# koide3/gtsam_points

Measured on AMD Instinct MI355X. Metric: point-correspondences/sec (VGICP linearize, 1M-pt source vs 2M-pt voxel map), higher is better.
Workload: dtype f64; 1 GPU; BASELINE configs[1]: single VGICP factor per GPU, 1M synthetic source pts vs 2M-pt GaussianVoxel; target_points=2000000, num_voxels=73733, num_buckets=262144, device_warmup_steps=14074

## Files before the change

gtsam_points_amd/csrc/gp_vgicp.hip:

```cpp
#include <algorithm>
#include <atomic>
#include <chrono>
#include <cmath>
#include <cstdlib>
#include <cstring>

#include "gp_host.hpp"
#include "gp_vgicp_tile.hpp"
#include "gp_vgicp_tile2.hpp"
#include "gp_vgicp_finalize.hpp"
#include "gp_vgicp_stream.hpp"

namespace gp {



template <int MODE>
struct ModeTraits {
  static constexpr int kAcc = MODE == MODE_ERR ? 2 : (MODE == MODE_LIN ? ACC_SIZE : ACCG_SIZE);
  static constexpr int kStride = MODE == MODE_LIN_GENERAL ? ACCG_STRIDE : ACC_STRIDE;
};

template <int MODE>
__device__ __forceinline__ void accumulate_point(const FactorDesc& f, const Pose& Tl, const Pose& Te, int i, double* acc) {
// ... 699 lines not shown
  return per * gp::kNumXCD;
}

bool poses_are_rigid(const double* poses_host, size_t F) {
  if (!poses_host) return false;
  for (size_t i = 0; i < F; i++)
    if (!gp::pose_is_rigid(poses_host + 16 * i)) return false;
  return true;
}

template <int MODE>
int launch_tiles(gp_vgicp_batch* b, const PoseSource& ps, double* partials) {
  if (b->num_tiles <= 0) return GP_OK;
  const int fam = MODE == gp::MODE_LIN_GENERAL ? GP_KERNEL_REFERENCE : b->family;
  const bool single_plan = b->planned;
  const int chunk = (fam == GP_KERNEL_REFERENCE || single_plan || (fam == GP_KERNEL_STREAM && ps.inl.use)) ? 0 : b->tuning.xcd_chunk;
  const dim3 grid_dim(grid_tiles(b->num_tiles, chunk)), block(gp::kBlockThreads);
  const gp::FactorDesc* fd = b->d_factors.as<gp::FactorDesc>();
  const gp::TileDesc* td = b->d_tiles.as<gp::TileDesc>();
  gp::InlinePoses inl = ps.inl;
  inl.stagger = b->tuning.stagger;
  inl.xcd_chunk = chunk;
  inl.tile_points = b->tile_points;
  inl.plan = b->plan;
  inl.trace = b->trace;
  const bool traced = b->trace != nullptr && inl.use && MODE == gp::MODE_LIN;
#define GP_ARGS grid_dim, block, 0, b->stream, fd, td, b->num_tiles, ps.d_lin, ps.d_eval, inl, partials
  if constexpr (MODE == gp::MODE_LIN_GENERAL) {
    hipLaunchKernelGGL(gp::vgicp_tile_kernel<MODE>, GP_ARGS);
  } else if (fam == GP_KERNEL_REFERENCE) {
    hipLaunchKernelGGL(gp::vgicp_tile_kernel<MODE>, GP_ARGS);
  } else if (fam == GP_KERNEL_STREAM) {
#define GP_LAUNCH_STREAM(NT, INL, SV, PK, TRACE) hipLaunchKernelGGL((gp::vgicp_stream_kernel<MODE, NT, INL, SV, PK, TRACE>), GP_ARGS)
#define GP_LAUNCH_STREAM_S(INL, SV)                                  \
  do {                                                               \
    if (b->packed) {                                                 \
      if (b->nt) GP_LAUNCH_STREAM(true, INL, SV, true, false);       \
      else GP_LAUNCH_STREAM(false, INL, SV, true, false);            \
    } else {                                                         \
      if (b->nt) GP_LAUNCH_STREAM(true, INL, SV, false, false);      \
      else GP_LAUNCH_STREAM(false, INL, SV, false, false);           \
    }                                                                \
  } while (0)
    if (traced && !b->any_sv) {
      if constexpr (MODE == gp::MODE_LIN) {
        if (b->packed) {
          if (b->nt) GP_LAUNCH_STREAM(true, true, false, true, true);
          else GP_LAUNCH_STREAM(false, true, false, true, true);
        } else {
          if (b->nt) GP_LAUNCH_STREAM(true, true, false, false, true);
          else GP_LAUNCH_STREAM(false, true, false, false, true);
        }
      }
    } else if (inl.use && MODE == gp::MODE_LIN && b->tuning.experiment && b->planned && b->packed && b->nt && !b->any_sv) {
      if constexpr (MODE == gp::MODE_LIN) {
        if (b->tuning.experiment == 1) hipLaunchKernelGGL((gp::vgicp_stream_kernel<MODE, true, true, false, true, false, 1>), GP_ARGS);
        else hipLaunchKernelGGL((gp::vgicp_stream_kernel<MODE, true, true, false, true, false, 2>), GP_ARGS);
      }
    } else if (inl.use) {
      if (b->any_sv) GP_LAUNCH_STREAM_S(true, true);
      else GP_LAUNCH_STREAM_S(true, false);
    } else {
      if (b->any_sv) GP_LAUNCH_STREAM_S(false, true);
      else GP_LAUNCH_STREAM_S(false, false);
    }
#undef GP_LAUNCH_STREAM_S
#undef GP_LAUNCH_STREAM
  } else {
#define GP_LAUNCH_PIPE(F32, PPT, GRID, LEAN, AHEAD) hipLaunchKernelGGL((gp::vgicp_pipeline_kernel<MODE, F32, PPT, GRID, false, LEAN, AHEAD>), GP_ARGS)
    if (fam == GP_KERNEL_HASHED) {
      GP_LAUNCH_PIPE(true, 4, false, false, false);
    } else if (fam == GP_KERNEL_GRID_F64) {
      GP_LAUNCH_PIPE(false, 4, true, false, false);
    } else {
      if constexpr (MODE == gp::MODE_LIN) GP_LAUNCH_PIPE(true, 4, true, true, true);
      else GP_LAUNCH_PIPE(true, 4, true, true, false);
    }
#undef GP_LAUNCH_PIPE
  }
#undef GP_ARGS
  GP_HIP(hipGetLastError());
  return GP_OK;
}

template <bool GENERAL>
int launch_finalize(gp_vgicp_batch* b, const PoseSource& ps, const double* partials, gp_linearized6* out_dev, gp::DoneFlags done = {}, int parts = 1) {
  if constexpr (GENERAL) {
    hipLaunchKernelGGL(gp::vgicp_finalize_kernel<true>, dim3((int)b->factors.size()), dim3(gp::kFinalizeThreads), 0, b->stream, b->d_factors.as<gp::FactorDesc>(),
                       ps.d_lin, ps.inl, partials, out_dev, done);
  } else {
    constexpr bool narrow = true;
    const int nparts = parts < 0 ? -parts : parts;
    if (nparts > 1 && narrow)
      hipLaunchKernelGGL(gp::vgicp_finalize_rigid_kernel<256>, dim3((int)b->factors.size() * nparts), dim3(256), 0, b->stream, b->d_factors.as<gp::FactorDesc>(), ps.d_lin,
                         ps.inl, partials, out_dev, done, parts);
    else
      hipLaunchKernelGGL(gp::vgicp_finalize_rigid_kernel<gp::kFinalizeThreads>, dim3((int)b->factors.size() * nparts), dim3(gp::kFinalizeThreads), 0, b->stream,
                         b->d_factors.as<gp::FactorDesc>(), ps.d_lin, ps.inl, partials, out_dev, done, parts);
  }
  GP_HIP(hipGetLastError());
  return GP_OK;
}

int launch_linearize(gp_vgicp_batch* b, const PoseSource& ps, gp_linearized6* out_dev, bool rigid, gp::DoneFlags done = {}, int parts = 1, bool timed = false) {
  if (b->factors.empty()) return GP_OK;
  double* partials = nullptr;
  GP_TRY(partials_ptr(b, &partials));
// ... 63 lines not shown
    b->tuning = f->tuning;
    const int rc = build_table(b);
    if (rc != GP_OK) {
      delete b;
      return rc;
    }
    f->self_batch = b;
  }
  if (table_is_stale(f->self_batch)) GP_TRY(build_table(f->self_batch));
  return GP_OK;
}

}

extern "C" {

static int apply_tuning(gp_vgicp_tuning* t, int key, int value) {
  switch (key) {
    case GP_TUNE_KERNEL:
      if (value != GP_KERNEL_REFERENCE && value != GP_KERNEL_HASHED && value != GP_KERNEL_GRID_F64 && value != GP_KERNEL_LOOKAHEAD && value != GP_KERNEL_STREAM)
        return gp::fail(GP_ERROR_INVALID_ARGUMENT, "GP_TUNE_KERNEL: one of GP_KERNEL_REFERENCE (0), _HASHED (2), _GRID_F64 (3), _LOOKAHEAD (8), _STREAM (12)");
      t->kernel = value;
      return GP_OK;
    case GP_TUNE_SOURCE_POLICY:
      if (value < 0 || value > 2) return gp::fail(GP_ERROR_INVALID_ARGUMENT, "GP_TUNE_SOURCE_POLICY: 0 (per batch), 1 (default cache policy), 2 (non-temporal)");
      t->source_policy = value;
      return GP_OK;
    case GP_TUNE_XCD_CHUNK:
      if (value < 0 || value > 4096) return gp::fail(GP_ERROR_INVALID_ARGUMENT, "GP_TUNE_XCD_CHUNK: 0 (contiguous eighths) .. 4096 tiles per run");
      t->xcd_chunk = value;
      return GP_OK;
    case GP_TUNE_STAGGER:
      if (value < 0 || value > 64) return gp::fail(GP_ERROR_INVALID_ARGUMENT, "GP_TUNE_STAGGER: 0..64 (x 512 clocks)");
      t->stagger = value;
      return GP_OK;
    case GP_TUNE_TILE_INTERLEAVE:
      t->tile_interleave = value ? 1 : 0;
      return GP_OK;
    case GP_TUNE_FUSED_FINALIZE:
      t->fused_finalize = value ? 1 : 0;
      return GP_OK;
    case GP_TUNE_MAX_WORKGROUPS:
      if (value < 8 || value > 1024) return gp::fail(GP_ERROR_INVALID_ARGUMENT, "GP_TUNE_MAX_WORKGROUPS: 8 .. 1024");
      t->max_wgs = value;
      return GP_OK;
    case GP_TUNE_TILE_CHUNKS:
      if (value < 0 || value > 64) return gp::fail(GP_ERROR_INVALID_ARGUMENT, "GP_TUNE_TILE_CHUNKS: 0 (automatic) .. 64 chunks per wave");
      t->tile_chunks = value;
      return GP_OK;
    case GP_TUNE_SOURCE_MIRROR:
      t->source_mirror = value ? 1 : 0;
      return GP_OK;
    case GP_TUNE_EXPERIMENT:
      if (value < 0 || value > 2) return gp::fail(GP_ERROR_INVALID_ARGUMENT, "GP_TUNE_EXPERIMENT: 0 (off), 1 (block-grid warm-up), 2 (f32 covariance rotation: breaks parity, timing only)");
      t->experiment = value;
      return GP_OK;
    case GP_TUNE_BALANCE:
      if (value < -1 || value > 600) return gp::fail(GP_ERROR_INVALID_ARGUMENT, "GP_TUNE_BALANCE: -1 (automatic), 0 (flat) .. 600 (per mille of the mean share per dispatch round)");
      t->balance = value;
      return GP_OK;
    default:
      if (key >= GP_TUNE_XCD_WEIGHT_0 && key < GP_TUNE_XCD_WEIGHT_0 + 8) {
        if (value < 500 || value > 1500) return gp::fail(GP_ERROR_INVALID_ARGUMENT, "GP_TUNE_XCD_WEIGHT_x: 500..1500 (per mille of the mean share)");
        t->xcd_weights[key - GP_TUNE_XCD_WEIGHT_0] = value;
        t->xcd_weights_set = true;
        return GP_OK;
      }
      return gp::fail(GP_ERROR_INVALID_ARGUMENT, "unknown GP_TUNE_* key");
  }
}

int gp_vgicp_batch_set_tuning(gp_vgicp_batch_t* b, int key, int value) {
  if (!b) return gp::fail(GP_ERROR_INVALID_ARGUMENT, "gp_vgicp_batch_set_tuning: null batch");
  if (key == GP_TUNE_TIMING) {
    b->timing = value != 0;
    return GP_OK;
  }
  if (key == GP_TUNE_TEST_ARRIVAL_SKEW) {
    b->arrived[0] += (unsigned long long)(value > 0 ? value : 0);
    if (b->d_factor_arrive.ptr && value > 0) {
      const unsigned long long v = 1ull << 40;
      GP_HIP(hipStreamSynchronize(b->stream));
      GP_HIP(hipMemcpy(b->d_factor_arrive.ptr, &v, sizeof(v), hipMemcpyHostToDevice));
    }
    return GP_OK;
  }
  GP_TRY(apply_tuning(&b->tuning, key, value));
  b->table_dirty = true;
  return GP_OK;
}

int gp_vgicp_batch_get_tuning(const gp_vgicp_batch_t* b, int key, int* value) {
  if (!b || !value) return gp::fail(GP_ERROR_INVALID_ARGUMENT, "gp_vgicp_batch_get_tuning: null");
  switch (key) {
    case GP_TUNE_KERNEL: *value = b->tuning.kernel; return GP_OK;
    case GP_TUNE_SOURCE_POLICY: *value = b->tuning.source_policy; return GP_OK;
    case GP_TUNE_XCD_CHUNK: *value = b->tuning.xcd_chunk; return GP_OK;
    case GP_TUNE_STAGGER: *value = b->tuning.stagger; return GP_OK;
    case GP_TUNE_TILE_INTERLEAVE: *value = b->tuning.tile_interleave; return GP_OK;
    case GP_TUNE_BALANCE: *value = b->tuning.balance; return GP_OK;
    case GP_TUNE_FUSED_FINALIZE: *value = b->tuning.fused_finalize; return GP_OK;
    case GP_TUNE_TILE_CHUNKS: *value = b->tuning.tile_chunks; return GP_OK;
    case GP_TUNE_EFFECTIVE_KERNEL: *value = b->table_dirty ? -1 : b->family; return GP_OK;
    case GP_TUNE_SOURCE_MIRROR: *value = b->tuning.source_mirror; return GP_OK;
    case GP_TUNE_EXPERIMENT: *value = b->tuning.experiment; return GP_OK;
    case GP_TUNE_EFFECTIVE_MIRROR: *value = b->table_dirty ? -1 : (b->packed ? 1 : 0); return GP_OK;
    default: return gp::fail(GP_ERROR_INVALID_ARGUMENT, "unknown GP_TUNE_* key");
// ... 756 lines not shown
```

gtsam_points_amd/csrc/gp_vgicp_stream.hpp:

```cpp
#pragma once

#include "gp_vgicp_finalize.hpp"
#include "gp_vgicp_tile2.hpp"

namespace gp {

template <bool NT>
__device__ __forceinline__ void chunk_dma12_row(const GP_GLOBAL char* urow, unsigned voff, char* slot) {
  chunk_dma12_pts<NT>(urow, voff, slot);
}

template <int N>
__device__ __forceinline__ void vm_wait_blk_n(v4i& blk) {
  static_assert(N == 0 || N == 3 || N == 4 || N == 5, "counts of the stream schedule");
  if constexpr (N == 0) asm volatile("s_waitcnt vmcnt(0)" : "+v"(blk) : : "memory");
  if constexpr (N == 3) asm volatile("s_waitcnt vmcnt(3)" : "+v"(blk) : : "memory");
  if constexpr (N == 4) asm volatile("s_waitcnt vmcnt(4)" : "+v"(blk) : : "memory");
  if constexpr (N == 5) asm volatile("s_waitcnt vmcnt(5)" : "+v"(blk) : : "memory");
}

struct WaveWork {
  size_t first;
  int n;
  int tail;
// ... 36 lines not shown
  for (int t0 = slice; t0 < row_count && wave < 4; t0 += 32 * kSlices) {
    double v[32];
#pragma unroll
    for (int k = 0; k < 32; k++) {
      const int t = t0 + k * kSlices;
      v[k] = t < row_count ? __builtin_bit_cast(double, __hip_atomic_load(base + (size_t)t * ACC_STRIDE, __ATOMIC_RELAXED, __HIP_MEMORY_SCOPE_AGENT)) : 0.0;
    }
#pragma unroll
    for (int w = 16; w > 0; w >>= 1) {
#pragma unroll
      for (int k = 0; k < w; k++) v[k] += v[k + w];
    }
    total += v[0];
  }
  total += __shfl_xor(total, 32, 64);
  if (tr && threadIdx.x == 0) tr[14] = __builtin_amdgcn_s_memrealtime();
  if (lane < 32 && wave < 4) wsum[wave * 32 + lane] = total;
  __syncthreads();
  if (wave != 0) return;
  double s = lane < 32 ? (wsum[lane] + wsum[64 + lane]) + (wsum[32 + lane] + wsum[96 + lane]) : 0.0;
  if (lane == 32) s = __builtin_bit_cast(double, t_rows);
  if (lane == 33) s = __builtin_bit_cast(double, __builtin_amdgcn_s_memrealtime());
  if (lane < 34) asm volatile("global_store_dwordx2 %0, %1, off sc0 sc1" : : "v"(out + lane), "v"(s) : "memory");
  asm volatile("s_waitcnt vmcnt(0)" ::: "memory");
  if (lane == 0) asm volatile("global_store_dwordx2 %0, %1, off sc0 sc1" : : "v"(flag), "v"(seq) : "memory");
  if (tr && lane == 0) tr[15] = __builtin_amdgcn_s_memrealtime();
}

__device__ __forceinline__ void finalize_part_error(const double* __restrict__ partials, const int row_begin, const int row_count, double* wsum, double* out,
                                                    unsigned long long* flag, const unsigned long long seq) {
  const int lane = threadIdx.x & 63, wave = threadIdx.x >> 6;
  const unsigned long long* base = reinterpret_cast<const unsigned long long*>(partials + (size_t)row_begin * ACC_STRIDE + ACC_ERR);
  double s = 0.0;
  for (int t = threadIdx.x; t < row_count && wave < 4; t += 256)
    s += __builtin_bit_cast(double, __hip_atomic_load(base + (size_t)t * ACC_STRIDE, __ATOMIC_RELAXED, __HIP_MEMORY_SCOPE_AGENT));
#pragma unroll
  for (int off = 32; off > 0; off >>= 1) s += __shfl_down(s, off, 64);
  if (lane == 0 && wave < 4) wsum[wave] = s;
  __syncthreads();
  if (threadIdx.x != 0) return;
  const double total = (wsum[0] + wsum[1]) + (wsum[2] + wsum[3]);
  asm volatile("global_store_dwordx2 %0, %1, off sc0 sc1\n\ts_waitcnt vmcnt(0)" : : "v"(out), "v"(total) : "memory");
  asm volatile("global_store_dwordx2 %0, %1, off sc0 sc1" : : "v"(flag), "v"(seq) : "memory");
}

template <int MODE, bool NT, bool INL, bool SV, bool PK, bool TRACE = false, int EXP = 0, int W = 4>
__global__ void __launch_bounds__(64 * W, 4) vgicp_stream_kernel(const FactorDesc* __restrict__ factors, const TileDesc* __restrict__ tiles, int num_tiles,
                                                               const double* __restrict__ poses_lin, const double* __restrict__ poses_eval, const InlinePoses inl,
                                                               double* __restrict__ partials) {
  static_assert(MODE == MODE_LIN || MODE == MODE_ERR, "rigid linearise and error evaluation");
  constexpr int NACC = MODE == MODE_ERR ? 2 : 32;
  constexpr int KC = PK ? 2 : 3;
  constexpr int K = 1 + KC + (SV ? 1 : 0);
  constexpr int kNrmSlotBytes = SV ? kPtsSlotBytes : 0;
  constexpr int kChunkSlotBytes = PK ? kCovSlotBytes : kPtsSlotBytes + kCovSlotBytes;
  constexpr int kRingBytes = 2 * kChunkSlotBytes + 2 * kNrmSlotBytes;
  constexpr int kWaveBytes = kRingBytes > kWaveLdsBytes ? kRingBytes : kWaveLdsBytes;
  static_assert(kWaveBytes >= kWaveLdsBytes, "the reduction needs 8.5 KB of the wave's region");
  static_assert(W * kWaveBytes <= 160 * 1024, "one workgroup's rings must fit the compute unit's LDS");
  __shared__ __attribute__((aligned(16))) char smem[W * kWaveBytes];
  const unsigned long long t_begin = INL ? __builtin_amdgcn_s_memrealtime() : 0ull;
  const int bx = blockIdx.x % kNumXCD, bq = blockIdx.x / kNumXCD;
  int tile_idx;
  FactorDesc f;
  WaveWork ww;
  int factor_idx = 0, row;
  int wgs_per_xcd = 0;
  const int wave = __builtin_amdgcn_readfirstlane(threadIdx.x >> 6);
  if constexpr (INL) {
    PlanFields pf = plan_fields(inl.plan, bx, bq);
    wgs_per_xcd = pf.gx;
    int tile_points = inl.tile_points, fn = inl.factor.n;
    const float* fpts = inl.factor.points;
    const float* fcov = inl.factor.covs;
    const float* fnrm = inl.factor.normals;
    const char* fpk = inl.factor.packed;
    asm volatile("" : "+s"(pf.nr), "+s"(pf.pre), "+s"(pf.lo), "+s"(pf.extra), "+s"(pf.xbegin), "+s"(pf.L), "+s"(pf.before_last), "+s"(pf.gx), "+s"(pf.tail), "+s"(tile_points),
                 "+s"(fn), "+s"(fpts), "+s"(fcov), "+s"(fnrm), "+s"(fpk));
    int begin, count;
    if (tile_points == 0) {
      tile_idx = bx * pf.gx + bq;
      plan_tile(pf, bx, bq, &begin, &count);
    } else {
      const int per = (num_tiles + kNumXCD - 1) / kNumXCD;
      tile_idx = bx * per + bq;
      if (bq >= per || tile_idx >= num_tiles) return;
      begin = tile_idx * tile_points;
      count = min(tile_points, fn - begin);
    }
    f = inl.factor;
    f.points = fpts;
    f.covs = fcov;
    f.normals = fnrm;
    f.packed = fpk;
    row = tile_idx;
    ww = split_tile<W>(begin, count, wave);
  } else {
    if (inl.xcd_chunk > 0) {
      const int c = inl.xcd_chunk;
      tile_idx = ((bq / c) * kNumXCD + bx) * c + (bq % c);
    } else {
      const int per = (num_tiles + kNumXCD - 1) / kNumXCD;
      tile_idx = bx * per + bq;
    }
    if (tile_idx >= num_tiles) return;
    const TileDesc tile = tiles[tile_idx];
    f = factors[tile.factor];
    factor_idx = tile.factor;
    row = tile.row;
    ww = split_tile<W>(__builtin_amdgcn_readfirstlane(tile.begin), __builtin_amdgcn_readfirstlane(tile.count), wave);
  }
  unsigned long long* trace = TRACE ? inl.trace : nullptr;
  GP_TRACE(0);
  if constexpr (INL && MODE == MODE_LIN) {
    if (inl.arrive && inl.rows_per_part > 0 && blockIdx.x < kNumXCD && threadIdx.x == 0)
      asm volatile("global_store_dwordx2 %0, %1, off sc0 sc1" : : "v"(inl.fin_out + (size_t)blockIdx.x * inl.fin_stride + 34), "v"(t_begin) : "memory");
  }
  if constexpr (TRACE) {
    if (trace && threadIdx.x == 0) {
      trace[(size_t)tile_idx * 16 + 10] = __builtin_amdgcn_s_memrealtime();
      trace[(size_t)tile_idx * 16 + 8] = __builtin_amdgcn_s_getreg(GP_GETREG_HW_ID);
      trace[(size_t)tile_idx * 16 + 9] = __builtin_amdgcn_s_getreg(GP_GETREG_XCC_ID);
    }
  }
  const int lane = threadIdx.x & 63;
  const int n = __builtin_amdgcn_readfirstlane(ww.n);
  const int tail = __builtin_amdgcn_readfirstlane(ww.tail);
  const size_t first = ww.first;
  char* wbase = smem + wave * kWaveBytes;
  auto pslot = [&](int par) { return PK ? wbase + par * kCovSlotBytes : wbase + par * kPtsSlotBytes; };
  auto nslot = [&](int par) { return PK ? wbase + 2 * kCovSlotBytes + par * kNrmSlotBytes : wbase + 2 * kPtsSlotBytes + par * kNrmSlotBytes; };
  auto cslot = [&](int par) { return PK ? wbase + par * kCovSlotBytes : wbase + 2 * kPtsSlotBytes + 2 * kNrmSlotBytes + par * kCovSlotBytes; };
  const GP_GLOBAL char* upts = PK ? uniform_ptr((const GP_GLOBAL char*)f.packed + (first >> 6) * (size_t)kPackedChunkBytes) : uniform_ptr((const GP_GLOBAL char*)as_global(f.points) + 12 * first);
  const GP_GLOBAL char* ucov = PK ? upts : uniform_ptr((const GP_GLOBAL char*)as_global(f.covs) + 36 * first);
  const GP_GLOBAL char* unrm = SV ? uniform_ptr((const GP_GLOBAL char*)as_global(f.normals) + 12 * first) : nullptr;
  const unsigned voff = (unsigned)lane * 12u;
  constexpr size_t kSrcChunkStride = PK ? (size_t)kPackedChunkBytes : (size_t)kChunkPoints * 12, kCovChunkStride = PK ? (size_t)kPackedChunkBytes : (size_t)kChunkPoints * 36;
  auto dma_head = [&](int j, int par) {
    chunk_dma12_pts<NT>(upts + (size_t)j * kSrcChunkStride, voff, pslot(par));
    if constexpr (SV) chunk_dma12_row<NT>(unrm + (size_t)j * (kChunkPoints * 12), voff, nslot(par));
  };
  auto dma_cov = [&](int j, int par) {
    if constexpr (PK) chunk_dma12_cov_packed<NT>(ucov + (size_t)j * kCovChunkStride, voff, cslot(par));
    else chunk_dma12_cov<NT>(ucov + (size_t)j * kCovChunkStride, voff, cslot(par));
  };

  if (n > 0) dma_head(0, 0);

  const Pose Tl = INL ? load_pose(inl.lin) : load_pose(poses_lin + 16 * (size_t)factor_idx);
  const Pose Te = MODE == MODE_ERR ? (INL ? load_pose(inl.eval) : load_pose(poses_eval + 16 * (size_t)factor_idx)) : Tl;
  const double leaf = uniform_f64(f.map.leaf), inv_leaf = uniform_f64(f.map.inv_leaf), half_leaf = uniform_f64(0.5 * f.map.leaf);
  const int glo0 = f.map.glo[0], glo1 = f.map.glo[1], glo2 = f.map.glo[2];
  const unsigned gd0 = __builtin_amdgcn_readfirstlane((unsigned)f.map.gdim[0]), gd1 = __builtin_amdgcn_readfirstlane((unsigned)f.map.gdim[1]), gd2 = (unsigned)f.map.gdim[2];
  const GP_GLOBAL char* gblocks = uniform_ptr((const GP_GLOBAL char*)f.map.gblocks);
  const GP_GLOBAL char* records = uniform_ptr((const GP_GLOBAL char*)f.map.records);

  v4i warm = {0, 0, 0, 0};
  if constexpr (EXP == 1) {
    const unsigned gbytes = gd0 * gd1 * gd2 * 16u;
#pragma unroll
    for (int k = 0; k < 4; k++) {
      const unsigned off = ((unsigned)(k * wgs_per_xcd + bq) * 256u + threadIdx.x) * 16u;
      if (off < gbytes) asm volatile("global_load_dwordx4 %0, %1, %2" : "+v"(warm) : "v"(off), "s"(gblocks) : "memory");
    }
  }
  double tvx, tvy, tvz;
  asm volatile("v_mov_b64 %0, %1" : "=v"(tvx) : "s"(Tl.tx));
  asm volatile("v_mov_b64 %0, %1" : "=v"(tvy) : "s"(Tl.ty));
  asm volatile("v_mov_b64 %0, %1" : "=v"(tvz) : "s"(Tl.tz));

  float acc[NACC];
#pragma unroll
  for (int k = 0; k < NACC; k++) acc[k] = 0.f;

  struct Ahead {
    v4i blk;
    float ex, ey, ez, qx, qy, qz;
    int pos;
  };
  auto front = [&](float pxf, float pyf, float pzf, float nxf, float nyf, float nzf, bool active, Ahead& P) {
#pragma clang fp contract(off)
    const double dx = (double)pxf, dy = (double)pyf, dz = (double)pzf;
    const double lx = __builtin_fma(Tl.r00, dx, __builtin_fma(Tl.r01, dy, __builtin_fma(Tl.r02, dz, tvx)));
    const double ly = __builtin_fma(Tl.r10, dx, __builtin_fma(Tl.r11, dy, __builtin_fma(Tl.r12, dz, tvy)));
    const double lz = __builtin_fma(Tl.r20, dx, __builtin_fma(Tl.r21, dy, __builtin_fma(Tl.r22, dz, tvz)));
    const double ux = lx * inv_leaf, uy = ly * inv_leaf, uz = lz * inv_leaf;
    const int cx = (int)__builtin_floor(ux), cy = (int)__builtin_floor(uy), cz = (int)__builtin_floor(uz);
    if constexpr (MODE == MODE_ERR) {
      const double ex_ = __builtin_fma(Te.r00, dx, __builtin_fma(Te.r01, dy, __builtin_fma(Te.r02, dz, Te.tx)));
      const double ey_ = __builtin_fma(Te.r10, dx, __builtin_fma(Te.r11, dy, __builtin_fma(Te.r12, dz, Te.ty)));
      const double ez_ = __builtin_fma(Te.r20, dx, __builtin_fma(Te.r21, dy, __builtin_fma(Te.r22, dz, Te.tz)));
      P.ex = (float)(__builtin_fma(-leaf, __builtin_amdgcn_fract(ux), half_leaf) + (lx - ex_));
      P.ey = (float)(__builtin_fma(-leaf, __builtin_amdgcn_fract(uy), half_leaf) + (ly - ey_));
      P.ez = (float)(__builtin_fma(-leaf, __builtin_amdgcn_fract(uz), half_leaf) + (lz - ez_));
      P.qx = P.qy = P.qz = 0.f;
    } else {
      P.ex = (float)__builtin_fma(-leaf, __builtin_amdgcn_fract(ux), half_leaf);
      P.ey = (float)__builtin_fma(-leaf, __builtin_amdgcn_fract(uy), half_leaf);
      P.ez = (float)__builtin_fma(-leaf, __builtin_amdgcn_fract(uz), half_leaf);
      P.qx = (float)lx;
      P.qy = (float)ly;
      P.qz = (float)lz;
    }
    bool live = active && finite3(pxf, pyf, pzf);
    if constexpr (SV) {
      const double nx = (double)nxf, ny = (double)nyf, nz = (double)nzf;
      const double tnx = __builtin_fma(Tl.r02, nz, __builtin_fma(Tl.r01, ny, Tl.r00 * nx)), tny = __builtin_fma(Tl.r12, nz, __builtin_fma(Tl.r11, ny, Tl.r10 * nx));
      const double tnz = __builtin_fma(Tl.r22, nz, __builtin_fma(Tl.r21, ny, Tl.r20 * nx));
      const double s = __builtin_fma(lz, tnz, __builtin_fma(ly, tny, lx * tnx));
      const double qq = __builtin_fma(lz, lz, __builtin_fma(ly, ly, lx * lx));
      if (s > 0.0 && s * s > (0.174 * 0.174) * qq) live = false;
    }
    const unsigned bx = (unsigned)((cx >> 2) - glo0), by = (unsigned)((cy >> 2) - glo1), bz = (unsigned)((cz >> 2) - glo2);
    const bool inbox = (bx < gd0) & (by < gd1) & (bz < gd2);
    const unsigned lin = inbox ? mad24s(mad24s(bz, gd1, by), gd0, bx) : 0u;
    P.pos = (inbox && live) ? (((cz & 3) << 4) | ((cy & 3) << 2) | (cx & 3)) : -1;
    grid_issue_s(gblocks, lin * 16u, P.blk);
  };
  auto front_ring = [&](int par, Ahead& P) {
    const v3f pt = *reinterpret_cast<const v3f*>(pslot(par) + 16 * lane);
    v3f nr = {0.f, 0.f, 0.f};
    if constexpr (SV) nr = *reinterpret_cast<const v3f*>(nslot(par) + 16 * lane);
    front(pt.x, pt.y, pt.z, nr.x, nr.y, nr.z, true, P);
  };
  auto back_issue = [&](const Ahead& P, v4f& head, v2d& c01, v2d& c23, v2d& c45) -> bool {
    const unsigned long long bits = ((unsigned long long)(unsigned)P.blk.y << 32) | (unsigned long long)(unsigned)P.blk.x;
    const int pos = P.pos < 0 ? 0 : P.pos;
    const bool hit = P.pos >= 0 && ((bits >> pos) & 1ull);
    const int idx = P.blk.z + __popcll(bits & ((1ull << pos) - 1ull));
    record_issue_s(records, hit ? (unsigned)idx << 6 : 0u, head, c01, c23, c45);
    return hit;
  };
  auto cov_ring = [&](int par, double* a) {
    if constexpr (PK) {
      const char* c = cslot(par) + 16 * lane;
      const v3f ca = *reinterpret_cast<const v3f*>(c + kPtsSlotBytes), cb = *reinterpret_cast<const v3f*>(c + 2 * kPtsSlotBytes);
      a[0] = (double)ca.x, a[1] = (double)ca.y, a[2] = (double)ca.z, a[3] = (double)cb.x, a[4] = (double)cb.y, a[5] = (double)cb.z;
    } else {
      const char* c = cslot(par) + 48 * lane;
      const v3f c0 = *reinterpret_cast<const v3f*>(c), c1 = *reinterpret_cast<const v3f*>(c + 16), c2 = *reinterpret_cast<const v3f*>(c + 32);
      const float c9[9] = {c0.x, c0.y, c0.z, c1.x, c1.y, c1.z, c2.x, c2.y, c2.z};
      load_cov6(c9, a);
    }
  };

  Ahead Pc;
  v4f head;
  v2d c01, c23, c45;
  double a[6];
  if (n > 0) {
    vm_wait<0>();
    if constexpr (EXP == 1) asm volatile("" : : "v"(warm));
    GP_TRACE(1);
    front_ring(0, Pc);
    dma_cov(0, 0);
    const bool has1 = n > 1;
    if (has1) dma_head(1, 1);
    else vm_wait<KC>();
    vm_wait_blk_n<K>(Pc.blk);
    GP_TRACE(2);
    bool hit = back_issue(Pc, head, c01, c23, c45);
    if (has1) dma_cov(1, 1);
    else asm volatile("s_waitcnt vmcnt(0)" ::: "memory");
    vm_wait_rec<KC>(head, c01, c23, c45);
    for (int j = 0;; j++) {
      const int par = j & 1;
      const bool more = j + 1 < n, more2 = j + 2 < n;
      Ahead Pn;
      if (more) front_ring(par ^ 1, Pn);
      cov_ring(par, a);
      if (more2) {
        asm volatile("s_waitcnt lgkmcnt(0)" ::: "memory");
        dma_head(j + 2, par);
        dma_cov(j + 2, par);
      }
      if (hit) accumulate_core2<MODE, EXP == 2>(Tl, a, c01, c23, c45, Pc.ex + head.x, Pc.ey + head.y, Pc.ez + head.z, Pc.qx, Pc.qy, Pc.qz, acc);
      if constexpr (TRACE) {
        if (j == 0) GP_TRACE(3);
        if (j == 1) GP_TRACE(5);
      }
      if (!more) break;
      if (!more2) asm volatile("s_waitcnt vmcnt(0)" ::: "memory");
      vm_wait_blk_n<K>(Pn.blk);
      if constexpr (TRACE) {
        if (j == 0) GP_TRACE(4);
      }
      hit = back_issue(Pn, head, c01, c23, c45);
      vm_wait_rec<0>(head, c01, c23, c45);
      Pc.ex = Pn.ex;
      Pc.ey = Pn.ey;
      Pc.ez = Pn.ez;
      Pc.qx = Pn.qx;
      Pc.qy = Pn.qy;
      Pc.qz = Pn.qz;
    }
    vm_wait<0>();
  }
  if (tail > 0) {
    const GP_GLOBAL float* points = as_global(f.points);
    const GP_GLOBAL float* covs = as_global(f.covs);
    const bool active = lane < tail;
    const size_t i = first + (size_t)n * kChunkPoints + (active ? lane : 0);
    v3f pt, nr = {0.f, 0.f, 0.f};
    v4f ca, cb;
    float cc;
    asm volatile(
      "global_load_dwordx3 %0, %4, off\n\t"
      "global_load_dwordx4 %1, %5, off\n\t"
      "global_load_dwordx4 %2, %5, off offset:16\n\t"
      "global_load_dword %3, %5, off offset:32\n\t"
      "s_waitcnt vmcnt(0)"
      : "=&v"(pt), "=&v"(ca), "=&v"(cb), "=&v"(cc)
      : "v"(points + 3 * i), "v"(covs + 9 * i)
      : "memory");
    if constexpr (SV) {
      const GP_GLOBAL float* normals = as_global(f.normals);
      asm volatile(
        "global_load_dwordx3 %0, %1, off\n\t"
        "s_waitcnt vmcnt(0)"
        : "=&v"(nr)
        : "v"(normals + 3 * i)
        : "memory");
    }
    const float c9[9] = {ca.x, ca.y, ca.z, ca.w, cb.x, cb.y, cb.z, cb.w, cc};
    Ahead P;
    front(pt.x, pt.y, pt.z, nr.x, nr.y, nr.z, active, P);
    vm_wait_blk_n<0>(P.blk);
    const bool hit = back_issue(P, head, c01, c23, c45);
    vm_wait_rec<0>(head, c01, c23, c45);
    load_cov6(c9, a);
    if (hit) accumulate_core2<MODE>(Tl, a, c01, c23, c45, P.ex + head.x, P.ey + head.y, P.ez + head.z, P.qx, P.qy, P.qz, acc);
  }

  GP_TRACE(6);
  constexpr int kRowStrideF = 66;
  static_assert(32 * kRowStrideF * 4 + 32 * 8 <= kWaveBytes, "f32 transposition buffer + wave sums must fit the wave's LDS region");
  float* wtf = reinterpret_cast<float*>(wbase);
  double* wsums = reinterpret_cast<double*>(wbase + kWaveBytes - 32 * 8);
  if constexpr (MODE == MODE_ERR) {
#pragma unroll
    for (int k = 0; k < 2; k++) {
      double v = (double)acc[k];
#pragma unroll
      for (int off = 32; off > 0; off >>= 1) v += __shfl_xor(v, off, 64);
      if (lane == 0) wsums[k] = v;
    }
  } else {
// ... 130 lines not shown
```

gtsam_points_amd/csrc/gp_vgicp_tile2.hpp:

```cpp
#pragma once

#include "gp_vgicp_tile.hpp"

namespace gp {

template <typename T>
__device__ __forceinline__ const GP_GLOBAL T* uniform_ptr(const GP_GLOBAL T* p) {
  const unsigned long long v = (unsigned long long)p;
  const unsigned lo = __builtin_amdgcn_readfirstlane((unsigned)v), hi = __builtin_amdgcn_readfirstlane((unsigned)(v >> 32));
  return (const GP_GLOBAL T*)(((unsigned long long)hi << 32) | lo);
}
__device__ __forceinline__ double uniform_f64(double x) {
  const unsigned long long v = __builtin_bit_cast(unsigned long long, x);
  const unsigned lo = __builtin_amdgcn_readfirstlane((unsigned)v), hi = __builtin_amdgcn_readfirstlane((unsigned)(v >> 32));
  return __builtin_bit_cast(double, ((unsigned long long)hi << 32) | lo);
}

constexpr int kPtsSlotBytes = 1024, kCovSlotBytes = 3072, kWaveLdsBytes = 8704;
static_assert(2 * kPtsSlotBytes + 2 * kCovSlotBytes <= kWaveLdsBytes, "ring must fit the wave's LDS region");

template <bool NT>
__device__ __forceinline__ void chunk_dma12_pts(const GP_GLOBAL char* upts, unsigned voff, char* pslot) {
  const unsigned lds_pts = (unsigned)(size_t)(GP_LDS char*)pslot;
  unsigned saved;
// ... 55 lines not shown
__device__ __forceinline__ void chunk_dma12_cov_packed(const GP_GLOBAL char* uchunk, unsigned voff, char* slot) {
  const unsigned lds_c1 = (unsigned)(size_t)(GP_LDS char*)slot + 256u, lds_c2 = lds_c1 + 256u;
  unsigned saved;
  if constexpr (NT) {
    asm volatile(
      "s_mov_b32 %0, m0\n\t"
      "s_mov_b32 m0, %3\n\t"
      "global_load_lds_dwordx3 %1, %2 offset:768 nt\n\t"
      "s_mov_b32 m0, %4\n\t"
      "global_load_lds_dwordx3 %1, %2 offset:1536 nt\n\t"
      "s_mov_b32 m0, %0"
      : "=&s"(saved)
      : "v"(voff), "s"(uchunk), "s"(lds_c1), "s"(lds_c2)
      : "memory");
  } else {
    asm volatile(
      "s_mov_b32 %0, m0\n\t"
      "s_mov_b32 m0, %3\n\t"
      "global_load_lds_dwordx3 %1, %2 offset:768\n\t"
      "s_mov_b32 m0, %4\n\t"
      "global_load_lds_dwordx3 %1, %2 offset:1536\n\t"
      "s_mov_b32 m0, %0"
      : "=&s"(saved)
      : "v"(voff), "s"(uchunk), "s"(lds_c1), "s"(lds_c2)
      : "memory");
  }
}

__device__ __forceinline__ unsigned mad24(unsigned a, unsigned b, unsigned c) {
  unsigned r;
  asm("v_mad_u32_u24 %0, %1, %2, %3" : "=v"(r) : "v"(a), "v"(b), "v"(c));
  return r;
}

__device__ __forceinline__ unsigned mad24s(unsigned a, unsigned b_uniform, unsigned c) {
  unsigned r;
  asm("v_mad_u32_u24 %0, %1, %2, %3" : "=v"(r) : "v"(a), "s"(b_uniform), "v"(c));
  return r;
}

__device__ __forceinline__ void grid_issue_s(const GP_GLOBAL char* base, unsigned off, v4i& blk) {
  asm volatile("global_load_dwordx4 %0, %1, %2" : "=&v"(blk) : "v"(off), "s"(base) : "memory");
}
__device__ __forceinline__ void record_issue_s(const GP_GLOBAL char* base, unsigned off, v4f& head, v2d& c01, v2d& c23, v2d& c45) {
  asm volatile(
    "global_load_dwordx4 %0, %4, %5\n\t"
    "global_load_dwordx4 %1, %4, %5 offset:16\n\t"
    "global_load_dwordx4 %2, %4, %5 offset:32\n\t"
    "global_load_dwordx4 %3, %4, %5 offset:48"
    : "=&v"(head), "=&v"(c01), "=&v"(c23), "=&v"(c45)
    : "v"(off), "s"(base)
    : "memory");
}
template <int N>
__device__ __forceinline__ void vm_wait() {
  static_assert(N >= 0 && N <= 8, "counts used by the schedules below");
  if constexpr (N == 0) asm volatile("s_waitcnt vmcnt(0)" ::: "memory");
  if constexpr (N == 1) asm volatile("s_waitcnt vmcnt(1)" ::: "memory");
  if constexpr (N == 2) asm volatile("s_waitcnt vmcnt(2)" ::: "memory");
  if constexpr (N == 3) asm volatile("s_waitcnt vmcnt(3)" ::: "memory");
  if constexpr (N == 4) asm volatile("s_waitcnt vmcnt(4)" ::: "memory");
  if constexpr (N == 7) asm volatile("s_waitcnt vmcnt(7)" ::: "memory");
  static_assert(N == 0 || N == 1 || N == 2 || N == 3 || N == 4 || N == 7, "add the count");
}
template <int N>
__device__ __forceinline__ void vm_wait_blk(v4i& blk) {
  if constexpr (N == 0) asm volatile("s_waitcnt vmcnt(0)" : "+v"(blk) : : "memory");
  if constexpr (N == 1) asm volatile("s_waitcnt vmcnt(1)" : "+v"(blk) : : "memory");
  if constexpr (N == 3) asm volatile("s_waitcnt vmcnt(3)" : "+v"(blk) : : "memory");
  if constexpr (N == 4) asm volatile("s_waitcnt vmcnt(4)" : "+v"(blk) : : "memory");
  static_assert(N == 0 || N == 1 || N == 3 || N == 4, "add the count");
}
template <int N>
__device__ __forceinline__ void vm_wait_rec(v4f& head, v2d& c01, v2d& c23, v2d& c45) {
  if constexpr (N == 0) asm volatile("s_waitcnt vmcnt(0)" : "+v"(head), "+v"(c01), "+v"(c23), "+v"(c45) : : "memory");
  if constexpr (N == 2) asm volatile("s_waitcnt vmcnt(2)" : "+v"(head), "+v"(c01), "+v"(c23), "+v"(c45) : : "memory");
  if constexpr (N == 3) asm volatile("s_waitcnt vmcnt(3)" : "+v"(head), "+v"(c01), "+v"(c23), "+v"(c45) : : "memory");
  if constexpr (N == 4) asm volatile("s_waitcnt vmcnt(4)" : "+v"(head), "+v"(c01), "+v"(c23), "+v"(c45) : : "memory");
  static_assert(N == 0 || N == 2 || N == 3 || N == 4, "add the count");
}

template <int MODE, bool ROT32 = false>
__device__ __forceinline__ void accumulate_core2(const Pose& Tl, const double* a, const v2d& c01, const v2d& c23, const v2d& c45, float RX, float RY, float RZ, float QX,
                                                 float QY, float QZ, float* acc) {
#pragma clang fp contract(off)
  float M0, M1, M2, M3, M4, M5;
  if constexpr (ROT32) {
    const float r00 = (float)Tl.r00, r01 = (float)Tl.r01, r02 = (float)Tl.r02, r10 = (float)Tl.r10, r11 = (float)Tl.r11, r12 = (float)Tl.r12, r20 = (float)Tl.r20,
                r21 = (float)Tl.r21, r22 = (float)Tl.r22;
    const float a00 = (float)a[0], a01 = (float)a[1], a02 = (float)a[2], a11 = (float)a[3], a12 = (float)a[4], a22 = (float)a[5];
    const auto d3 = [](float x0, float y0, float x1, float y1, float x2, float y2) { return __builtin_fmaf(x2, y2, __builtin_fmaf(x1, y1, x0 * y0)); };
    const float rc00 = d3(r00, a00, r01, a01, r02, a02), rc01 = d3(r00, a01, r01, a11, r02, a12), rc02 = d3(r00, a02, r01, a12, r02, a22);
    const float rc10 = d3(r10, a00, r11, a01, r12, a02), rc11 = d3(r10, a01, r11, a11, r12, a12), rc12 = d3(r10, a02, r11, a12, r12, a22);
    const float rc20 = d3(r20, a00, r21, a01, r22, a02), rc21 = d3(r20, a01, r21, a11, r22, a12), rc22 = d3(r20, a02, r21, a12, r22, a22);
    const double s00 = c01.x + (double)d3(rc00, r00, rc01, r01, rc02, r02), s01 = c01.y + (double)d3(rc00, r10, rc01, r11, rc02, r12);
    const double s02 = c23.x + (double)d3(rc00, r20, rc01, r21, rc02, r22), s11 = c23.y + (double)d3(rc10, r10, rc11, r11, rc12, r12);
    const double s12 = c45.x + (double)d3(rc10, r20, rc11, r21, rc12, r22), s22 = c45.y + (double)d3(rc20, r20, rc21, r21, rc22, r22);
    const double i00 = __builtin_fma(s11, s22, -(s12 * s12)), i01 = __builtin_fma(s02, s12, -(s01 * s22)), i02 = __builtin_fma(s01, s12, -(s02 * s11));
    const double det = __builtin_fma(s02, i02, __builtin_fma(s01, i01, s00 * i00));
    double x = __builtin_amdgcn_rcp(det);
    x = x * __builtin_fma(-det, x, 2.0);
    M0 = (float)(i00 * x);
    M1 = (float)(i01 * x);
    M2 = (float)(i02 * x);
    M3 = (float)(__builtin_fma(s00, s22, -(s02 * s02)) * x);
    M4 = (float)(__builtin_fma(s01, s02, -(s00 * s12)) * x);
    M5 = (float)(__builtin_fma(s00, s11, -(s01 * s01)) * x);
  } else {
    const double a00 = a[0], a01 = a[1], a02 = a[2], a11 = a[3], a12 = a[4], a22 = a[5];
    const auto dot3 = [](double x0, double y0, double x1, double y1, double x2, double y2) { return __builtin_fma(x2, y2, __builtin_fma(x1, y1, x0 * y0)); };
    const auto dot3p = [](double c, double x0, double y0, double x1, double y1, double x2, double y2) { return __builtin_fma(x2, y2, __builtin_fma(x1, y1, __builtin_fma(x0, y0, c))); };
    const double rc00 = dot3(Tl.r00, a00, Tl.r01, a01, Tl.r02, a02), rc01 = dot3(Tl.r00, a01, Tl.r01, a11, Tl.r02, a12), rc02 = dot3(Tl.r00, a02, Tl.r01, a12, Tl.r02, a22);
    const double rc10 = dot3(Tl.r10, a00, Tl.r11, a01, Tl.r12, a02), rc11 = dot3(Tl.r10, a01, Tl.r11, a11, Tl.r12, a12), rc12 = dot3(Tl.r10, a02, Tl.r11, a12, Tl.r12, a22);
    const double rc20 = dot3(Tl.r20, a00, Tl.r21, a01, Tl.r22, a02), rc21 = dot3(Tl.r20, a01, Tl.r21, a11, Tl.r22, a12), rc22 = dot3(Tl.r20, a02, Tl.r21, a12, Tl.r22, a22);
    const double s00 = dot3p(c01.x, rc00, Tl.r00, rc01, Tl.r01, rc02, Tl.r02);
    const double s01 = dot3p(c01.y, rc00, Tl.r10, rc01, Tl.r11, rc02, Tl.r12);
// ... 54 lines not shown
```

Measured before the change: 50.22 billion point-correspondences/s.

## Stage voxel record gathers through LDS DMA to overlap with next chunk's loads

```diff
diff --git a/gtsam_points_amd/csrc/gp_vgicp.hip b/gtsam_points_amd/csrc/gp_vgicp.hip
--- a/gtsam_points_amd/csrc/gp_vgicp.hip
+++ b/gtsam_points_amd/csrc/gp_vgicp.hip
@@ -775,7 +775,17 @@
           else GP_LAUNCH_STREAM(false, true, false, false, true);
         }
       }
-    } else if (inl.use && MODE == gp::MODE_LIN && b->tuning.experiment && b->planned && b->packed && b->nt && !b->any_sv) {
+    } else if (b->tuning.experiment == 3 && b->packed && !b->any_sv) {
+#define GP_LAUNCH_UNSTAGED(NT, INL) hipLaunchKernelGGL((gp::vgicp_stream_kernel<MODE, NT, INL, false, true, false, 3>), GP_ARGS)
+      if (inl.use) {
+        if (b->nt) GP_LAUNCH_UNSTAGED(true, true);
+        else GP_LAUNCH_UNSTAGED(false, true);
+      } else {
+        if (b->nt) GP_LAUNCH_UNSTAGED(true, false);
+        else GP_LAUNCH_UNSTAGED(false, false);
+      }
+#undef GP_LAUNCH_UNSTAGED
+    } else if (inl.use && MODE == gp::MODE_LIN && (b->tuning.experiment == 1 || b->tuning.experiment == 2) && b->planned && b->packed && b->nt && !b->any_sv) {
       if constexpr (MODE == gp::MODE_LIN) {
         if (b->tuning.experiment == 1) hipLaunchKernelGGL((gp::vgicp_stream_kernel<MODE, true, true, false, true, false, 1>), GP_ARGS);
         else hipLaunchKernelGGL((gp::vgicp_stream_kernel<MODE, true, true, false, true, false, 2>), GP_ARGS);
@@ -945,7 +955,9 @@
       t->source_mirror = value ? 1 : 0;
       return GP_OK;
     case GP_TUNE_EXPERIMENT:
-      if (value < 0 || value > 2) return gp::fail(GP_ERROR_INVALID_ARGUMENT, "GP_TUNE_EXPERIMENT: 0 (off), 1 (block-grid warm-up), 2 (f32 covariance rotation: breaks parity, timing only)");
+      if (value < 0 || value > 3)
+        return gp::fail(GP_ERROR_INVALID_ARGUMENT, "GP_TUNE_EXPERIMENT: 0 (off), 1 (block-grid warm-up), 2 (f32 covariance rotation: breaks parity, timing only), "
+                                                   "3 (packed stream without the record stage)");
       t->experiment = value;
       return GP_OK;
     case GP_TUNE_BALANCE:
diff --git a/gtsam_points_amd/csrc/gp_vgicp_stream.hpp b/gtsam_points_amd/csrc/gp_vgicp_stream.hpp
--- a/gtsam_points_amd/csrc/gp_vgicp_stream.hpp
+++ b/gtsam_points_amd/csrc/gp_vgicp_stream.hpp
@@ -112,9 +112,10 @@
   constexpr int NACC = MODE == MODE_ERR ? 2 : 32;
   constexpr int KC = PK ? 2 : 3;
   constexpr int K = 1 + KC + (SV ? 1 : 0);
+  constexpr bool STAGE = PK && !SV && EXP != 3;
   constexpr int kNrmSlotBytes = SV ? kPtsSlotBytes : 0;
   constexpr int kChunkSlotBytes = PK ? kCovSlotBytes : kPtsSlotBytes + kCovSlotBytes;
-  constexpr int kRingBytes = 2 * kChunkSlotBytes + 2 * kNrmSlotBytes;
+  constexpr int kRingBytes = 2 * kChunkSlotBytes + 2 * kNrmSlotBytes + (STAGE ? kStageBytes : 0);
   constexpr int kWaveBytes = kRingBytes > kWaveLdsBytes ? kRingBytes : kWaveLdsBytes;
   static_assert(kWaveBytes >= kWaveLdsBytes, "the reduction needs 8.5 KB of the wave's region");
   static_assert(W * kWaveBytes <= 160 * 1024, "one workgroup's rings must fit the compute unit's LDS");
@@ -191,6 +192,7 @@
   auto pslot = [&](int par) { return PK ? wbase + par * kCovSlotBytes : wbase + par * kPtsSlotBytes; };
   auto nslot = [&](int par) { return PK ? wbase + 2 * kCovSlotBytes + par * kNrmSlotBytes : wbase + 2 * kPtsSlotBytes + par * kNrmSlotBytes; };
   auto cslot = [&](int par) { return PK ? wbase + par * kCovSlotBytes : wbase + 2 * kPtsSlotBytes + 2 * kNrmSlotBytes + par * kCovSlotBytes; };
+  char* const stage = wbase + 2 * kChunkSlotBytes;
   const GP_GLOBAL char* upts = PK ? uniform_ptr((const GP_GLOBAL char*)f.packed + (first >> 6) * (size_t)kPackedChunkBytes) : uniform_ptr((const GP_GLOBAL char*)as_global(f.points) + 12 * first);
   const GP_GLOBAL char* ucov = PK ? upts : uniform_ptr((const GP_GLOBAL char*)as_global(f.covs) + 36 * first);
   const GP_GLOBAL char* unrm = SV ? uniform_ptr((const GP_GLOBAL char*)as_global(f.normals) + 12 * first) : nullptr;
@@ -291,6 +293,14 @@
     record_issue_s(records, hit ? (unsigned)idx << 6 : 0u, head, c01, c23, c45);
     return hit;
   };
+  auto back_issue_stage = [&](const Ahead& P) -> bool {
+    const unsigned long long bits = ((unsigned long long)(unsigned)P.blk.y << 32) | (unsigned long long)(unsigned)P.blk.x;
+    const int pos = P.pos < 0 ? 0 : P.pos;
+    const bool hit = P.pos >= 0 && ((bits >> pos) & 1ull);
+    const int idx = P.blk.z + __popcll(bits & ((1ull << pos) - 1ull));
+    record_dma_s(records, hit ? (unsigned)idx << 6 : 0u, stage);
+    return hit;
+  };
   auto cov_ring = [&](int par, double* a) {
     if constexpr (PK) {
       const char* c = cslot(par) + 16 * lane;
@@ -319,40 +329,85 @@
     else vm_wait<KC>();
     vm_wait_blk_n<K>(Pc.blk);
     GP_TRACE(2);
-    bool hit = back_issue(Pc, head, c01, c23, c45);
-    if (has1) dma_cov(1, 1);
-    else asm volatile("s_waitcnt vmcnt(0)" ::: "memory");
-    vm_wait_rec<KC>(head, c01, c23, c45);
-    for (int j = 0;; j++) {
-      const int par = j & 1;
-      const bool more = j + 1 < n, more2 = j + 2 < n;
-      Ahead Pn;
-      if (more) front_ring(par ^ 1, Pn);
-      cov_ring(par, a);
-      if (more2) {
-        asm volatile("s_waitcnt lgkmcnt(0)" ::: "memory");
-        dma_head(j + 2, par);
-        dma_cov(j + 2, par);
-      }
-      if (hit) accumulate_core2<MODE, EXP == 2>(Tl, a, c01, c23, c45, Pc.ex + head.x, Pc.ey + head.y, Pc.ez + head.z, Pc.qx, Pc.qy, Pc.qz, acc);
-      if constexpr (TRACE) {
-        if (j == 0) GP_TRACE(3);
-        if (j == 1) GP_TRACE(5);
-      }
-      if (!more) break;
-      if (!more2) asm volatile("s_waitcnt vmcnt(0)" ::: "memory");
-      vm_wait_blk_n<K>(Pn.blk);
-      if constexpr (TRACE) {
-        if (j == 0) GP_TRACE(4);
-      }
-      hit = back_issue(Pn, head, c01, c23, c45);
-      vm_wait_rec<0>(head, c01, c23, c45);
-      Pc.ex = Pn.ex;
-      Pc.ey = Pn.ey;
-      Pc.ez = Pn.ez;
-      Pc.qx = Pn.qx;
-      Pc.qy = Pn.qy;
-      Pc.qz = Pn.qz;
+    if constexpr (STAGE) {
+      static_assert(K - KC == 1, "the stage schedule counts one head row per chunk (packed stream, no normals)");
+      bool hit = back_issue_stage(Pc);
+      if (has1) dma_cov(1, 1);
+      for (int j = 0;; j++) {
+        const int par = j & 1;
+        const bool more = j + 1 < n, more2 = j + 2 < n;
+        Ahead Pn;
+        bool hit_n = false;
+        if (more) {
+          vm_wait<4 + KC>();
+          front_ring(par ^ 1, Pn);
+          vm_wait<KC + 1>();
+          record_from_stage(stage, lane, head, c01, c23, c45);
+          cov_ring(par, a);
+          asm volatile("s_waitcnt lgkmcnt(0)" ::: "memory");
+          if (more2) dma_head(j + 2, par);
+          else asm volatile("s_waitcnt vmcnt(0)" ::: "memory");
+          vm_wait_blk<1>(Pn.blk);
+          if constexpr (TRACE) {
+            if (j == 0) GP_TRACE(4);
+          }
+          hit_n = back_issue_stage(Pn);
+          if (more2) dma_cov(j + 2, par);
+        } else {
+          vm_wait<0>();
+          record_from_stage(stage, lane, head, c01, c23, c45);
+          cov_ring(par, a);
+        }
+        if (hit) accumulate_core2<MODE, EXP == 2>(Tl, a, c01, c23, c45, Pc.ex + head.x, Pc.ey + head.y, Pc.ez + head.z, Pc.qx, Pc.qy, Pc.qz, acc);
+        if constexpr (TRACE) {
+          if (j == 0) GP_TRACE(3);
+          if (j == 1) GP_TRACE(5);
+        }
+        if (!more) break;
+        hit = hit_n;
+        Pc.ex = Pn.ex;
+        Pc.ey = Pn.ey;
+        Pc.ez = Pn.ez;
+        Pc.qx = Pn.qx;
+        Pc.qy = Pn.qy;
+        Pc.qz = Pn.qz;
+      }
+    } else {
+      bool hit = back_issue(Pc, head, c01, c23, c45);
+      if (has1) dma_cov(1, 1);
+      else asm volatile("s_waitcnt vmcnt(0)" ::: "memory");
+      vm_wait_rec<KC>(head, c01, c23, c45);
+      for (int j = 0;; j++) {
+        const int par = j & 1;
+        const bool more = j + 1 < n, more2 = j + 2 < n;
+        Ahead Pn;
+        if (more) front_ring(par ^ 1, Pn);
+        cov_ring(par, a);
+        if (more2) {
+          asm volatile("s_waitcnt lgkmcnt(0)" ::: "memory");
+          dma_head(j + 2, par);
+          dma_cov(j + 2, par);
+        }
+        if (hit) accumulate_core2<MODE, EXP == 2>(Tl, a, c01, c23, c45, Pc.ex + head.x, Pc.ey + head.y, Pc.ez + head.z, Pc.qx, Pc.qy, Pc.qz, acc);
+        if constexpr (TRACE) {
+          if (j == 0) GP_TRACE(3);
+          if (j == 1) GP_TRACE(5);
+        }
+        if (!more) break;
+        if (!more2) asm volatile("s_waitcnt vmcnt(0)" ::: "memory");
+        vm_wait_blk_n<K>(Pn.blk);
+        if constexpr (TRACE) {
+          if (j == 0) GP_TRACE(4);
+        }
+        hit = back_issue(Pn, head, c01, c23, c45);
+        vm_wait_rec<0>(head, c01, c23, c45);
+        Pc.ex = Pn.ex;
+        Pc.ey = Pn.ey;
+        Pc.ez = Pn.ez;
+        Pc.qx = Pn.qx;
+        Pc.qy = Pn.qy;
+        Pc.qz = Pn.qz;
+      }
     }
     vm_wait<0>();
   }
diff --git a/gtsam_points_amd/csrc/gp_vgicp_tile2.hpp b/gtsam_points_amd/csrc/gp_vgicp_tile2.hpp
--- a/gtsam_points_amd/csrc/gp_vgicp_tile2.hpp
+++ b/gtsam_points_amd/csrc/gp_vgicp_tile2.hpp
@@ -131,6 +131,33 @@
     : "v"(off), "s"(base)
     : "memory");
 }
+constexpr int kStageBytes = 4096;
+__device__ __forceinline__ void record_dma_s(const GP_GLOBAL char* base, unsigned off, char* stage) {
+  const unsigned s0 = (unsigned)(size_t)(GP_LDS char*)stage, s1 = s0 + 1024u - 16u, s2 = s0 + 2048u - 32u, s3 = s0 + 3072u - 48u;
+  unsigned saved;
+  asm volatile(
+    "s_mov_b32 %0, m0\n\t"
+    "s_mov_b32 m0, %3\n\t"
+    "global_load_lds_dwordx4 %1, %2\n\t"
+    "s_mov_b32 m0, %4\n\t"
+    "global_load_lds_dwordx4 %1, %2 offset:16\n\t"
+    "s_mov_b32 m0, %5\n\t"
+    "global_load_lds_dwordx4 %1, %2 offset:32\n\t"
+    "s_mov_b32 m0, %6\n\t"
+    "global_load_lds_dwordx4 %1, %2 offset:48\n\t"
+    "s_mov_b32 m0, %0"
+    : "=&s"(saved)
+    : "v"(off), "s"(base), "s"(s0), "s"(s1), "s"(s2), "s"(s3)
+    : "memory");
+}
+__device__ __forceinline__ void record_from_stage(const char* stage, int lane, v4f& head, v2d& c01, v2d& c23, v2d& c45) {
+  const char* s = stage + 16 * lane;
+  head = *reinterpret_cast<const v4f*>(s);
+  c01 = *reinterpret_cast<const v2d*>(s + 1024);
+  c23 = *reinterpret_cast<const v2d*>(s + 2048);
+  c45 = *reinterpret_cast<const v2d*>(s + 3072);
+}
+
 template <int N>
 __device__ __forceinline__ void vm_wait() {
   static_assert(N >= 0 && N <= 8, "counts used by the schedules below");
@@ -139,8 +166,9 @@
   if constexpr (N == 2) asm volatile("s_waitcnt vmcnt(2)" ::: "memory");
   if constexpr (N == 3) asm volatile("s_waitcnt vmcnt(3)" ::: "memory");
   if constexpr (N == 4) asm volatile("s_waitcnt vmcnt(4)" ::: "memory");
+  if constexpr (N == 6) asm volatile("s_waitcnt vmcnt(6)" ::: "memory");
   if constexpr (N == 7) asm volatile("s_waitcnt vmcnt(7)" ::: "memory");
-  static_assert(N == 0 || N == 1 || N == 2 || N == 3 || N == 4 || N == 7, "add the count");
+  static_assert(N == 0 || N == 1 || N == 2 || N == 3 || N == 4 || N == 6 || N == 7, "add the count");
 }
 template <int N>
 __device__ __forceinline__ void vm_wait_blk(v4i& blk) {
```

Measured after the change: 50.46 billion point-correspondences/s (median of 6 runs). No clear change (+0.5%).
